# schmidtjonathan/pnmol-experiments

Measured on AMD Instinct MI355X. Metric: filter steps/sec, 1D heat N=512 nu=2 (white-noise EK1 predict+update), higher is better.
Workload: dtype f64; 1 GPU; 1-D heat equation, N=512 mesh, IWP(nu=2) EK1, Dirichlet, dt=2^-7, one problem per GPU (kappa sweep), D=1536, m=514; steps_in_one_call=4975, valid=True, problems_per_gpu=1

## Files before the change

pnmol-experiments_amd/csrc/pnmol_hip.hip:

```cpp
#include <hip/hip_runtime.h>

#include <algorithm>
#include <chrono>
#include <cmath>
#include <cstdio>
#include <cstdlib>
#include <cstring>
#include <string>
#include <utility>
#include <atomic>
#include <vector>

#include "pnmol_hip.h"
#include "pnmol_internal.hpp"

namespace {

constexpr int TLD = NB + 1;
typedef double d4 __attribute__((ext_vector_type(4)));

struct MeasModel {
    const int* ell_col;
    const double* ell_val;
    int w, d, m, dp, mp;
    double c0, c1;
};

constexpr int HW = 4;

struct HRow {
    int idx[HW + 1];
    double cf[HW + 1];
};

__device__ __forceinline__ void h_row_load(const MeasModel& mm, int i, HRow& r) {
    r.idx[0] = (i < mm.d) ? mm.dp + i : 0;
    r.cf[0] = (i < mm.d) ? mm.c1 : 0.0;
#pragma unroll
    for (int e = 0; e < HW; ++e) {
        const int cidx = (e < mm.w) ? mm.ell_col[e * mm.mp + i] : -1;
        const double val = (e < mm.w) ? mm.ell_val[e * mm.mp + i] : 0.0;
        r.idx[e + 1] = cidx >= 0 ? cidx : 0;
        r.cf[e + 1] = cidx >= 0 ? mm.c0 * val : 0.0;
    }
}

template <typename XT>
__device__ __forceinline__ double h_row_dot(const MeasModel& mm, int i, const XT* x) {
    double v = 0.0;
    if (i < mm.d) v = mm.c1 * x[mm.dp + i];
    for (int e = 0; e < mm.w; ++e) {
        const int cidx = mm.ell_col[e * mm.mp + i];
        if (cidx >= 0) v += mm.c0 * mm.ell_val[e * mm.mp + i] * x[cidx];
    }
    return v;
}

template <int W, typename XT>
__device__ __forceinline__ double h_row_dot_w(const HRow& r, const XT* __restrict__ x) {
    double xv[W + 1];
#pragma unroll
    for (int e = 0; e <= W; ++e) xv[e] = x[r.idx[e]];
    double v = r.cf[0] * xv[0];
#pragma unroll
    for (int e = 1; e <= W; ++e) v += r.cf[e] * xv[e];
    return v;
}

struct RoleArgs {
    IwpConsts c;
    int dp;
    const double* min;
    double* mpred;
    const double* shift;
    double* G;
    double* zbuf;
    MeasModel mm;
    int* flags;
    int nflags;
};

template <int N>
__device__ __forceinline__ void predict_vectors(double* mpl, int tid, const IwpConsts& c, int dp, const double* __restrict__ min,
                                                double* __restrict__ mpred, const double* __restrict__ shift,
                                                double* __restrict__ G, double* __restrict__ zbuf, const MeasModel& mm,
                                                int* __restrict__ flags, int nflags) {
    const long Dp = (long)N * dp;
    for (int e = tid; e < nflags; e += 256) flags[e] = 0;
    for (int j = tid; j < dp; j += 256) {
        double x[N];
#pragma unroll
        for (int a = 0; a < N; ++a) x[a] = c.ts[a] * min[a * dp + j];
#pragma unroll
        for (int a = 0; a < N; ++a) {
            double sacc = 0.0;
#pragma unroll
            for (int q = 0; q < N; ++q) sacc += c.A1[a * MAXN + q] * x[q];
            mpl[a * dp + j] = sacc;
            mpred[a * dp + j] = sacc;
        }
    }
    __syncthreads();
    for (int i = tid; i < mm.mp; i += 256) {
        const double v = (i < mm.m) ? h_row_dot(mm, i, mpl) + shift[i] : 0.0;
        G[((long)mm.mp + Dp) * mm.mp + i] = v;
        zbuf[i] = v;
    }
}

template <int N, typename PT>
__device__ __forceinline__ void predict_tile(const PT* __restrict__ Pin, PT* __restrict__ Pout, const double* __restrict__ Kg,
                                             const IwpConsts& c, int dp, int j, int k) {
    const long Dp = (long)N * dp;
    double X[N][N];
#pragma unroll
    for (int a = 0; a < N; ++a)
#pragma unroll
        for (int b = 0; b < N; ++b) X[a][b] = c.ts[a] * c.ts[b] * Pin[((long)a * dp + j) * Dp + (long)b * dp + k];
    const double kjk = Kg[(long)j * dp + k];
    double T[N][N];
#pragma unroll
    for (int a = 0; a < N; ++a)
#pragma unroll
        for (int e = 0; e < N; ++e) {
            double sacc = 0.0;
#pragma unroll
            for (int q = 0; q < N; ++q) sacc += c.A1[a * MAXN + q] * X[q][e];
            T[a][e] = sacc;
        }
#pragma unroll
    for (int a = 0; a < N; ++a)
#pragma unroll
        for (int b = 0; b < N; ++b) {
            double sacc = c.Q1[a * MAXN + b] * kjk;
#pragma unroll
            for (int e = 0; e < N; ++e) sacc += T[a][e] * c.A1[b * MAXN + e];
            Pout[((long)a * dp + j) * Dp + (long)b * dp + k] = (PT)sacc;
        }
}

template <int N>
__global__ __launch_bounds__(256) void k_predict(const void* __restrict__ Pin, void* __restrict__ Pout,
                                                 const double* __restrict__ Kg, IwpConsts c, int dp,
                                                 const double* __restrict__ min, double* __restrict__ mpred,
                                                 const double* __restrict__ shift, double* __restrict__ G,
                                                 double* __restrict__ zbuf, MeasModel mm, int* __restrict__ ctr,
                                                 int* __restrict__ flags, int nflags, int p32) {
    if (blockIdx.y == 0) {
        if (blockIdx.x != 0) return;
        extern __shared__ double mpl[];
        const int tid = threadIdx.y * 32 + threadIdx.x;
        predict_vectors<N>(mpl, tid, c, dp, min, mpred, shift, G, zbuf, mm, flags, nflags);
        if (tid == 0) *ctr += 1;
        return;
    }
    const int k = blockIdx.x * 32 + threadIdx.x;
    const int j = (blockIdx.y - 1) * 8 + threadIdx.y;
    if (p32) predict_tile<N>(static_cast<const float*>(Pin), static_cast<float*>(Pout), Kg, c, dp, j, k);
    else predict_tile<N>(static_cast<const double*>(Pin), static_cast<double*>(Pout), Kg, c, dp, j, k);
}

template <typename PT>
__device__ __forceinline__ double s_entry(const PT* __restrict__ Ppred, long Dp, const MeasModel& mm, int ip, int i,
                                          const double* __restrict__ rdiag, const double* __restrict__ Rdense) {
    if (ip >= mm.m || i >= mm.m) return (ip == i) ? 1.0 : 0.0;
    double v = 0.0;
    if (ip < mm.d) v = mm.c1 * h_row_dot(mm, i, Ppred + (long)(mm.dp + ip) * Dp);
    for (int e = 0; e < mm.w; ++e) {
        const int cidx = mm.ell_col[e * mm.mp + ip];
        if (cidx >= 0) v += mm.c0 * mm.ell_val[e * mm.mp + ip] * h_row_dot(mm, i, Ppred + (long)cidx * Dp);
    }
    if (ip == i) v += rdiag[i];
    if (Rdense) v += Rdense[(long)ip * mm.mp + i];
    return v;
}

template <int W, typename PT>
__device__ __forceinline__ double s_entry_w(const PT* __restrict__ Ppred, long Dp, const MeasModel& mm,
                                            const HRow& rrow , const HRow& rcol , int ip, int i,
                                            const double* __restrict__ rdiag, const double* __restrict__ Rdense) {
    if (ip >= mm.m || i >= mm.m) return (ip == i) ? 1.0 : 0.0;
    double t[W + 1];
#pragma unroll
    for (int e = 0; e <= W; ++e) t[e] = h_row_dot_w<W>(rcol, Ppred + (long)rrow.idx[e] * Dp);
    double v = rrow.cf[0] * t[0];
#pragma unroll
    for (int e = 1; e <= W; ++e) v += rrow.cf[e] * t[e];
    if (ip == i) v += rdiag[i];
    if (Rdense) v += Rdense[(long)ip * mm.mp + i];
    return v;
}

__device__ __forceinline__ double bcast_lane(double x, int src) {
    const int lo = __builtin_amdgcn_readlane(__double2loint(x), src);
    const int hi = __builtin_amdgcn_readlane(__double2hiint(x), src);
    return __hiloint2double(hi, lo);
}


struct Diag4Lds {
    double x0[4][64];
    double x1[8][64];
    double la[8][64];
    double n01[4][64];
    double piv[NB];
// ... 253 lines not shown
template <typename PT>
__device__ __forceinline__ void front_block_tiled(const PT* __restrict__ Ppred, double* __restrict__ G,
                                                  const double* __restrict__ rdiag, const double* __restrict__ Rdense,
                                                  const MeasModel& mm, long Dp, int fb) {
    const int tid = threadIdx.x, mp = mm.mp;
    const bool narrow = mm.w <= HW;
    const int nP = (int)(Dp / 8);
    if (fb < nP) {
        const long y0 = (long)fb * 8;
        for (int i = tid; i < mp; i += 256) {
            if (i >= mm.m) {
#pragma unroll
                for (int q = 0; q < 8; ++q) G[((long)mp + y0 + q) * mp + i] = 0.0;
                continue;
            }
            double v[8];
            if (narrow) {
                HRow rc;
                h_row_load(mm, i, rc);
#pragma unroll
                for (int q = 0; q < 8; ++q) v[q] = h_row_dot_w<HW>(rc, Ppred + (y0 + q) * Dp);
            } else {
#pragma unroll
                for (int q = 0; q < 8; ++q) v[q] = h_row_dot(mm, i, Ppred + (y0 + q) * Dp);
            }
#pragma unroll
            for (int q = 0; q < 8; ++q) G[((long)mp + y0 + q) * mp + i] = v[q];
        }
        return;
    }
    int t = fb - nP;
    int I = (int)((sqrt(8.0 * t + 1.0) - 1.0) * 0.5);
    while ((I + 1) * (I + 2) / 2 <= t) ++I;
    while (I * (I + 1) / 2 > t) --I;
    const int J = t - I * (I + 1) / 2;
    const int i = J * NB + (tid & 31);
    HRow rc;
    if (narrow && i < mm.m) h_row_load(mm, i, rc);
#pragma unroll
    for (int q = 0; q < 4; ++q) {
        const int ip = I * NB + (tid >> 5) + 8 * q;
        double v;
        if (narrow && ip < mm.m && i < mm.m) {
            HRow rr;
            h_row_load(mm, ip, rr);
            v = s_entry_w<HW>(Ppred, Dp, mm, rr, rc, ip, i, rdiag, Rdense);
        } else {
            v = s_entry(Ppred, Dp, mm, ip, i, rdiag, Rdense);
        }
        G[(long)ip * mp + i] = v;
    }
}

__global__ void k_set_identity(double* __restrict__ Gi, int mp) {
    const int q = blockIdx.x * blockDim.x + threadIdx.x;
    if (q < mp) Gi[(long)q * mp + q] = 1.0;
}

__global__ __launch_bounds__(256) void k_front(const void* __restrict__ Ppred, double* __restrict__ G,
                                               const double* __restrict__ rdiag, const double* __restrict__ Rdense,
                                               MeasModel mm, long Dp, int p32) {
    if (p32) front_block(static_cast<const float*>(Ppred), G, rdiag, Rdense, mm, Dp, blockIdx.x, blockIdx.y);
    else front_block(static_cast<const double*>(Ppred), G, rdiag, Rdense, mm, Dp, blockIdx.x, blockIdx.y);
}

__global__ __launch_bounds__(256) void k_front_s(double* __restrict__ G, const double* __restrict__ rdiag,
                                                 const double* __restrict__ Rdense, MeasModel mm) {
    const int i = blockIdx.x * 256 + threadIdx.x, ip = blockIdx.y, mp = mm.mp;
    if (i >= mp || i >= (ip / NB + 1) * NB) return;
    double v;
    if (ip >= mm.m || i >= mm.m) {
        v = (ip == i) ? 1.0 : 0.0;
    } else {
        const double* PHt = G + (long)mp * mp;
        v = 0.0;
        if (ip < mm.d) v = mm.c1 * PHt[(long)(mm.dp + ip) * mp + i];
        for (int e = 0; e < mm.w; ++e) {
            const int cidx = mm.ell_col[e * mp + ip];
            if (cidx >= 0) v += mm.c0 * mm.ell_val[e * mp + ip] * PHt[(long)cidx * mp + i];
        }
        if (ip == i) v += rdiag[i];
        if (Rdense) v += Rdense[(long)ip * mp + i];
    }
    G[(long)ip * mp + i] = v;
}

constexpr int SWEEP_SPIN_LIMIT = 1 << 18;
#ifdef PNMOL_SWEEP_STAMP
__device__ long long pnmol_sweep_stamp[512][8];
#define SWEEP_STAMP(slot) do { if (tid == 0 && L.stamp_id < 256) pnmol_sweep_stamp[L.stamp_id][slot] = wall_clock64(); } while (0)
#define SWEEP_STAMP_L(slot) do { if (l == 0 && L.stamp_id < 256) pnmol_sweep_stamp[L.stamp_id][slot] = wall_clock64(); } while (0)
#ifndef PNMOL_SWEEP_TRACE_WG
#define PNMOL_SWEEP_TRACE_WG 16
#endif
#define SWEEP_TRACE(j, slot) do { if (tid == 0 && L.stamp_id == PNMOL_SWEEP_TRACE_WG) pnmol_sweep_stamp[256 + (j)][slot] = wall_clock64(); } while (0)
#define SWEEP_TRACE_W2(j, slot) do { if (w == 2 && l == 0 && L.stamp_id == PNMOL_SWEEP_TRACE_WG) pnmol_sweep_stamp[320 + (j)][slot] = wall_clock64(); } while (0)
#define SWEEP_TRACE_VM(j, slot) do { asm volatile("s_waitcnt vmcnt(0)" ::: "memory"); SWEEP_TRACE(j, slot); } while (0)
#define CHAIN_TRACE(J, slot) do { if (tid == 0) pnmol_sweep_stamp[384 + (J)][slot] = wall_clock64(); } while (0)
#define CHAIN_TRACE_W(J, slot, wave) do { if (l == 0 && w == (wave)) pnmol_sweep_stamp[384 + (J)][slot] = wall_clock64(); } while (0)
#define CHAIN_TRACE_CLK(J, slot) do { if (tid == 0) pnmol_sweep_stamp[384 + (J)][slot] = clock64(); } while (0)
#define PNMOL_DD_DBG 1
#define DD_TRACE(j, slot) do { if (tid == 0 && pair == 60) pnmol_sweep_stamp[448 + (j)][slot] = wall_clock64(); } while (0)
#else
#define DD_TRACE(j, slot) do {} while (0)
#define CHAIN_TRACE_CLK(J, slot) do {} while (0)
#define SWEEP_TRACE_VM(j, slot) do {} while (0)
// ... 1729 lines not shown
    __syncthreads();
    if (w >= 2) return;
    {
        const double* rd = smem + w * C::RED;
#pragma unroll
        for (int a = 0; a < N; ++a)
#pragma unroll
            for (int b = 0; b < N; ++b)
#pragma unroll
                for (int r = 0; r < 4; ++r) acc[a][b][r] += rd[((a * N + b) * 4 + r) * 64 + l];
    }
    __syncthreads();
    if (w == 0)
        downdate_finish<N, 0>(acc, smem, Ppred, Pout, var, dp, Dp, J, K, l);
    else
        downdate_finish<N, 1>(acc, smem, Ppred, Pout, var, dp, Dp, J, K, l);
}

__global__ __launch_bounds__(256) void k_fill_q(void* __restrict__ Qf, const double* __restrict__ Kg, IwpConsts c, int n,
                                                int dp, int p32) {
    const long Dp = (long)n * dp;
    const long e = (long)blockIdx.x * 256 + threadIdx.x;
    if (e >= Dp * Dp) return;
    const long row = e / Dp, col = e % Dp;
    const int a = (int)(row / dp), j = (int)(row % dp), b = (int)(col / dp), k = (int)(col % dp);
    const double v = c.Q1[a * MAXN + b] * Kg[(long)j * dp + k];
    if (p32) static_cast<float*>(Qf)[e] = (float)v;
    else static_cast<double*>(Qf)[e] = v;
}

__global__ __launch_bounds__(256) void k_ttt(const double* __restrict__ T, double* __restrict__ C, int mp) {
    __shared__ double sa[16][17], sb[16][17];
    const int tx = threadIdx.x & 15, ty = threadIdx.x >> 4;
    const int i = blockIdx.y * 16 + ty, k = blockIdx.x * 16 + tx;
    double acc = 0.0;
    for (int q0 = 0; q0 < mp; q0 += 16) {
        sa[ty][tx] = T[(long)(blockIdx.y * 16 + ty) * mp + q0 + tx];
        sb[ty][tx] = T[(long)(blockIdx.x * 16 + ty) * mp + q0 + tx];
        __syncthreads();
#pragma unroll
        for (int q = 0; q < 16; ++q) acc += sa[ty][q] * sb[tx][q];
        __syncthreads();
    }
    C[(long)i * mp + k] = acc;
}

template <int N, bool ROLE>
__global__ __launch_bounds__(256) void k_readout(const double* __restrict__ mean, const double* __restrict__ var,
                                                 double* __restrict__ means_base, double* __restrict__ stds_base,
                                                 double s0, int d, const double* __restrict__ part,
                                                 double* __restrict__ rec_base, int mp, int* __restrict__ ctr,
                                                 RoleArgs ra, int* __restrict__ tickets, int rblocks,
                                                 const void* __restrict__ Ppred, const double* __restrict__ rdiag,
                                                 const double* __restrict__ Rdense, int p32) {
    if constexpr (ROLE) {
        if ((int)blockIdx.x > rblocks) {
            const int fb = blockIdx.x - rblocks - 1;
            if (p32) front_block_tiled(static_cast<const float*>(Ppred), ra.G, rdiag, Rdense, ra.mm, (long)N * ra.dp, fb);
            else front_block_tiled(static_cast<const double*>(Ppred), ra.G, rdiag, Rdense, ra.mm, (long)N * ra.dp, fb);
            return;
        }
    }
    const int slot = __builtin_amdgcn_readfirstlane(*ctr) - 1;
    if constexpr (ROLE) {
        if ((int)blockIdx.x == rblocks) {
            extern __shared__ double mpl[];
            predict_vectors<N>(mpl, threadIdx.x, ra.c, ra.dp, ra.min, ra.mpred, ra.shift, ra.G, ra.zbuf, ra.mm, ra.flags,
                               ra.nflags);
            if (threadIdx.x == 0) {
                int spins = 0;
                while (__hip_atomic_load(tickets, __ATOMIC_RELAXED, __HIP_MEMORY_SCOPE_AGENT) < rblocks &&
                       ++spins < (1 << 22)) __builtin_amdgcn_s_sleep(1);
                *ctr = slot + 2;
                __hip_atomic_store(tickets, 0, __ATOMIC_RELAXED, __HIP_MEMORY_SCOPE_AGENT);
            }
            return;
        }
        __syncthreads();
        if (threadIdx.x == 0) atomicAdd(tickets, 1);
    }
    const int j = blockIdx.x * blockDim.x + threadIdx.x;
    double* means = means_base ? means_base + (size_t)slot * d : nullptr;
    double* stds = stds_base ? stds_base + (size_t)slot * d : nullptr;
    double* rec = rec_base + 4 * (size_t)slot;
    if (j < d) {
        if (means) means[j] = s0 * mean[j];
        if (stds) stds[j] = s0 * sqrt(fmax(var[j], 0.0));
    }
    if (blockIdx.x == 0) {
        __shared__ double sred[3][4];
        double a[3] = {0.0, 0.0, 0.0};
        for (int i = threadIdx.x; i < mp; i += 256)
#pragma unroll
            for (int q = 0; q < 3; ++q) a[q] += part[q * mp + i];
#pragma unroll
        for (int q = 0; q < 3; ++q)
#pragma unroll
            for (int o = 32; o > 0; o >>= 1) a[q] += __shfl_xor(a[q], o);
        if ((threadIdx.x & 63) == 0)
            for (int q = 0; q < 3; ++q) sred[q][threadIdx.x >> 6] = a[q];
        __syncthreads();
        if (threadIdx.x < 3) rec[threadIdx.x] = sred[threadIdx.x][0] + sred[threadIdx.x][1] + sred[threadIdx.x][2] + sred[threadIdx.x][3];
    }
}

__global__ __launch_bounds__(256) void k_poison(double* __restrict__ F, long nF, double* __restrict__ Linv, long nL,
                                                double* __restrict__ hs, long nH) {
    const double bad = __longlong_as_double(0x7ff8dead0000beefLL);
    const long stride = (long)gridDim.x * 256;
    for (long e = (long)blockIdx.x * 256 + threadIdx.x; e < nF; e += stride) F[e] = bad;
    for (long e = (long)blockIdx.x * 256 + threadIdx.x; e < nL; e += stride) {
        const int r = (int)((e / NB) % NB), c = (int)(e % NB);
        if (!(r < 16 && c >= 16)) Linv[e] = bad;
    }
    for (long e = (long)blockIdx.x * 256 + threadIdx.x; e < nH; e += stride) hs[e] = bad;
}

__global__ void k_operator_diagonal(double* __restrict__ ell_val, const double* __restrict__ base_val,
                                    const int* __restrict__ slot, const double* __restrict__ op ,
                                    double* __restrict__ shift, int d, int mp) {
    const int i = blockIdx.x * blockDim.x + threadIdx.x;
// ... 199 lines not shown
    static const int mode = [] {
        const char* e = std::getenv("PNMOL_HIP_SWEEP_XL");
        return e ? (std::atoi(e) != 0 ? 1 : 0) : -1;
    }();
    return mode;
}
constexpr int MAX_DEVICES = 64;
std::atomic<int> live_rl_filters[MAX_DEVICES];
template <int N, bool FUSED>
void launch_sweep(unsigned grid, hipStream_t st, const double* G, double* F, double* Linv, int ld, int CB, int RT, int* flags,
                  int* info, const int* ctr, const DowndateArgs& dd, int* claim, double* hs, int lenient, int home,
                  bool wskip = false) {
    const bool xl = home >= 0;
    const unsigned rgrid = grid + (unsigned)w_split_count(RT, CB);
    unsigned xgrid = 8u * (unsigned)(CB - 1 + s_split_count(CB, true)) + 1u;
    for (unsigned left = rgrid - (unsigned)CB; left > 0; ++xgrid)
        if (xgrid % 8u != 0u) --left;
    xgrid += (unsigned)(xl ? home : 0);
    if (sweep_rl_enabled() && CB <= 9) {
        if (xl) k_sweep_rl<N, FUSED, 9, true><<<xgrid, 256, 0, st>>>(G, F, Linv, ld, CB, RT, flags, info, ctr, dd, hs, lenient, home);
        else k_sweep_rl<N, FUSED, 9, false><<<rgrid + 1, 256, 0, st>>>(G, F, Linv, ld, CB, RT, flags, info, ctr, dd, hs, lenient, home);
    } else if (sweep_rl_enabled() && CB <= 17) {
        if (xl) k_sweep_rl<N, FUSED, 17, true><<<xgrid, 256, 0, st>>>(G, F, Linv, ld, CB, RT, flags, info, ctr, dd, hs, lenient, home);
        else k_sweep_rl<N, FUSED, 17, false><<<rgrid + 1, 256, 0, st>>>(G, F, Linv, ld, CB, RT, flags, info, ctr, dd, hs, lenient, home);
    }
    else
        k_sweep<N, FUSED><<<grid, 256, 0, st>>>(G, F, Linv, ld, CB, RT, flags, info, ctr, dd, claim, hs, lenient, wskip ? 1 : 0);
}

inline bool short_last_panel() {
    static const int on = [] {
        const char* e = std::getenv("PNMOL_HIP_SHORT_LAST");
        return e ? std::atoi(e) : 1;
    }();
    return on != 0;
}
template <int N>
int launch_step(pnmol_filter* f, const double* Pin, const double* min, double frame_dt, double dt, double* Pout,
                double* mout, double* varout, bool record, StepKind kind) {
    pnmol_ctx* ctx = f->ctx;
    hipStream_t st = ctx->stream;
    IwpConsts c = f->iwp;
    for (int a = 0; a < f->n; ++a) {
        const double so = frame_dt == 0.0 ? 1.0 : nordsieck_scale(f->nu, a, frame_dt);
        c.ts[a] = so / nordsieck_scale(f->nu, a, dt);
    }
    MeasModel mm{f->ell_col, f->ell_val, f->ellw, f->d, f->m, f->dp, f->mp,
                 nordsieck_scale(f->nu, 0, dt), nordsieck_scale(f->nu, 1, dt)};
    const int dp = f->dp, mp = f->mp;
    const long Dp = f->Dp;

    if (kind != STEP_STEADY)
        k_predict<N><<<dim3(dp / 32, dp / 8 + 1), dim3(32, 8), sizeof(double) * Dp, st>>>(
        Pin, f->Ppred, f->Kg, c, dp, min, f->mpred, f->shift, f->G, f->zbuf, mm, f->ctr, f->flags, f->nflags, f->p32);
    if (kind != STEP_STEADY) {
        if (f->ellw > HW) {
            k_front<<<dim3((mp + 255) / 256, (unsigned)Dp), 256, 0, st>>>(f->Ppred, f->G, f->rdiag, f->Rdense, mm, Dp, f->p32);
            k_front_s<<<dim3((mp + 255) / 256, (unsigned)mp), 256, 0, st>>>(f->G, f->rdiag, f->Rdense, mm);
        } else {
            k_front<<<dim3((mp + 255) / 256, (unsigned)(Dp + mp)), 256, 0, st>>>(f->Ppred, f->G, f->rdiag, f->Rdense, mm, Dp, f->p32);
        }
    }
    const long rowI0 = (long)mp + Dp + NB;
    const double* W = f->F + (long)mp * mp;
    const bool have_sq = (f->Sqinv != nullptr && f->sq_dt == dt);
    VecArgs va{f->mpred, f->F + ((long)mp + Dp) * mp, f->F + rowI0 * mp, f->zbuf, have_sq ? f->Sqinv : nullptr,
               mout, f->part};
    const int nreal = f->m - NB * (f->CB - 1);
    DowndateArgs dd{f->Ppred, Pout, varout, dp, 0, va, kind == STEP_FULL ? nullptr : f->Ppred, f->Kg, f->last_ctr, {}, {}, f->p32,
                    (nreal < 8 && short_last_panel()) ? nreal : 0};
    std::memcpy(dd.A1, f->iwp.A1, sizeof(dd.A1));
    std::memcpy(dd.Q1, f->iwp.Q1, sizeof(dd.Q1));
    if (f->sweep_mode == 2) {
        const int t32 = dp / NB, pairs = t32 * (t32 + 1) / 2;
        dd.vrows = 0;
        if constexpr (N <= 3)
            launch_sweep<N, true>(f->RT + pairs, st, f->G, f->F, f->Linv, mp, f->CB, f->RT, f->flags, f->info, f->ctr, dd,
                                  f->flags + f->RT + f->CB + 1, f->hs_scratch, f->p32 ? 2 : 0, f->xcd_home);
    } else {
        if (f->w_gemm) {
            launch_sweep<N, false>(2 * f->CB + 1, st, f->G, f->F, f->Linv, mp, f->CB, f->RT, f->flags, f->info, f->ctr, dd,
                                   f->flags + f->RT + f->CB + 1, f->hs_scratch, f->p32 ? 2 : 0, f->xcd_home, true);
            const int nI = (int)(Dp / BDT), nt = nI * (mp / BDT);
            k_w_gemm<<<8 * ((nt + 7) / 8), 256, 0, st>>>(f->G + (long)mp * mp, f->F + rowI0 * mp, f->F + (long)mp * mp, mp, nI, nt);
        } else
        launch_sweep<N, false>(f->RT, st, f->G, f->F, f->Linv, mp, f->CB, f->RT, f->flags, f->info, f->ctr, dd,
                               f->flags + f->RT + f->CB + 1, f->hs_scratch, f->p32 ? 2 : 0, f->xcd_home);
        const int tiles = dp / 16;
        const int vrows = (int)(((Dp + mp + 3) / 4 + tiles - 1) / tiles);
        if (f->dd_big) {
            const int T = (int)(Dp / BDT), nt = T * (T + 1) / 2;
            if (f->p32)
                k_downdate_big<float><<<8 * ((nt + 7) / 8), 256, 0, st>>>(reinterpret_cast<const float*>(f->Ppred), W,
                                                                          reinterpret_cast<float*>(Pout), varout, Dp, mp, nt);
            else
                k_downdate_big<double><<<8 * ((nt + 7) / 8), 256, 0, st>>>(static_cast<const double*>(f->Ppred), W, Pout, varout,
                                                                           Dp, mp, nt);
            k_vecops<<<dim3(tiles, vrows), 256, 0, st>>>(va, W, mp, Dp, tiles);
        } else {
            k_downdate<N><<<dim3(tiles, tiles + vrows), 256, 0, st>>>(f->Ppred, W, Pout, varout, dp, mp, 0, mp / 8, va);
        }
    }
    IwpConsts cn = f->iwp;
    for (int a = 0; a < MAXN; ++a) cn.ts[a] = 1.0;
    RoleArgs ra{cn, dp, mout, f->mpred, f->shift, f->G, f->zbuf, mm, f->flags, f->nflags};
    const unsigned rblocks = (f->d + 255) / 256;
    if (kind == STEP_FULL)
        k_readout<N, false><<<rblocks, 256, 0, st>>>(mout, varout, record ? f->rec_means : nullptr,
                                                    record ? f->rec_stds : nullptr, nordsieck_scale(f->nu, 0, dt), f->d,
                                                    f->part, f->rec, mp, f->ctr, ra, f->tickets, (int)rblocks, f->Ppred, f->rdiag,
                                                    f->Rdense, f->p32);
    else
        k_readout<N, true><<<rblocks + 1 + (unsigned)front_tiled_blocks(Dp, mp), 256, sizeof(double) * Dp, st>>>(
            mout, varout, record ? f->rec_means : nullptr, record ? f->rec_stds : nullptr, nordsieck_scale(f->nu, 0, dt),
            f->d, f->part, f->rec, mp, f->ctr, ra, f->tickets, (int)rblocks, f->Ppred, f->rdiag, f->Rdense, f->p32);
    hipError_t e = hipGetLastError();
    if (e != hipSuccess) {
        ctx->err = std::string("kernel launch: ") + hipGetErrorString(e);
        return -2;
    }
    return 0;
}

int dispatch_step(pnmol_filter* f, const double* Pin, const double* min, double frame_dt, double dt, double* Pout,
                  double* mout, double* varout, bool record, StepKind kind = STEP_FULL) {
    switch (f->n) {
        case 2: return launch_step<2>(f, Pin, min, frame_dt, dt, Pout, mout, varout, record, kind);
        case 3: return launch_step<3>(f, Pin, min, frame_dt, dt, Pout, mout, varout, record, kind);
        case 4: return launch_step<4>(f, Pin, min, frame_dt, dt, Pout, mout, varout, record, kind);
    }
    return -1;
}

int loop_step(pnmol_filter* f, const double* Pin, const double* min, double frame_dt, double dt, double* Pout, double* mout,
              double* varout, StepKind kind, bool keep = true) {
    if (has_term(f)) {
        if (int rc = pnmol_reaction_enqueue(f, min, frame_dt, dt, true)) return rc;
    }
    if (int rc = dispatch_step(f, Pin, min, frame_dt, dt, Pout, mout, varout, true, kind)) return rc;
    return keep ? pnmol_record_enqueue(f, Pout, mout, varout) : 0;
}

void drop_graphs(pnmol_filter* f) {
    for (auto& g : f->graphs)
        if (g.exec) (void)hipGraphExecDestroy(g.exec);
    f->graphs.clear();
}

int get_graph(pnmol_filter* f, double* P0, double* M0, double* P1, double* M1, double* var, double dt, int nsteps,
              hipGraphExec_t* out) {
    pnmol_ctx* ctx = f->ctx;
    const bool have_sq = (f->Sqinv != nullptr && f->sq_dt == dt);
    for (auto& g : f->graphs)
        if (g.P0 == P0 && g.P1 == P1 && g.var == var && g.dt == dt && g.nsteps == nsteps && g.have_sq == have_sq &&
            g.fused == fused_loop(f)) {
            *out = g.exec;
            return 0;
        }
    if (f->graphs.size() >= 8) drop_graphs(f);
    hipGraph_t graph = nullptr;
    HIPCHK(ctx, hipStreamBeginCapture(ctx->stream, hipStreamCaptureModeThreadLocal));
    int rc = 0;
    for (int it = 0; it < nsteps && rc == 0; ++it)
        rc = (it & 1) ? loop_step(f, P1, M1, dt, dt, P0, M0, var, fused_loop(f) ? STEP_STEADY : STEP_FULL)
                      : loop_step(f, P0, M0, dt, dt, P1, M1, var, fused_loop(f) ? STEP_STEADY : STEP_FULL);
    hipError_t e = hipStreamEndCapture(ctx->stream, &graph);
    if (rc != 0 || e != hipSuccess) {
        if (graph) (void)hipGraphDestroy(graph);
// ... 387 lines not shown
    FCHK(hipMalloc(&f->ell_val, sizeof(double) * eval.size()));
    FCHK(hipMalloc(&f->Kg, sizeof(double) * Kg.size()));
    FCHK(hipMalloc(&f->rdiag, sizeof(double) * mp));
    FCHK(hipMalloc(&f->shift, sizeof(double) * mp));
    FCHK(hipMalloc(&f->G, sizeof(double) * tall));
    FCHK(hipMalloc(&f->F, sizeof(double) * tall));
    FCHK(hipMalloc(&f->Linv, sizeof(double) * (size_t)f->CB * NB * NB));
    FCHK(hipMemset(f->Linv, 0, sizeof(double) * (size_t)f->CB * NB * NB));
    FCHK(hipMalloc(&f->Ppred, f->psz * (size_t)Dp * Dp));
    FCHK(hipMalloc(&f->tmpP, f->psz * (size_t)Dp * Dp));
    FCHK(hipMalloc(&f->mpred, sizeof(double) * Dp));
    FCHK(hipMalloc(&f->tmpMean, sizeof(double) * Dp));
    FCHK(hipMalloc(&f->var, sizeof(double) * Dp));
    FCHK(hipMalloc(&f->zbuf, sizeof(double) * mp));
    FCHK(hipMalloc(&f->part, sizeof(double) * 3 * mp));
    FCHK(hipMalloc(&f->ctr, sizeof(int)));
    {
        const int h1 = 1;
        FCHK(hipMalloc(&f->one, sizeof(int)));
        FCHK(hipMalloc(&f->info_err, sizeof(int)));
        FCHK(hipMemcpy(f->one, &h1, sizeof(int), hipMemcpyHostToDevice));
    }
    if (const char* gc = std::getenv("PNMOL_HIP_GRAPH_CHUNK")) f->graph_chunk = std::atoi(gc) / 2 * 2;
    f->sweep_mode = sweep_mode;
    if (f->sweep_mode == 2 && n > 3) f->sweep_mode = 1;
    {
        const char* e = std::getenv("PNMOL_HIP_DD_BIG");
        const bool fits = f->Dp % BDT == 0 && f->mp % BDK == 0 && (!f->p32 || f->sweep_mode == 2);
        const bool want = e ? std::atoi(e) != 0 : (f->Dp >= 8192 && f->CB > 17);
        if (fits && want) {
            f->dd_big = 1;
            f->sweep_mode = 1;
            const char* g = std::getenv("PNMOL_HIP_W_GEMM");
            f->w_gemm = (g ? std::atoi(g) != 0 : 1) && f->mp % BDT == 0 && f->CB > 17;
        }
    }
    {
        static std::atomic<int> next_home[MAX_DEVICES];
        const bool rl = sweep_rl_enabled() && f->CB <= 17;
        if (rl) {
            const int dv = ctx->device % MAX_DEVICES;
            const int others = live_rl_filters[dv].fetch_add(1);
            f->counted = true;
            const bool xl = sweep_xl_mode() < 0 ? others == 0 : sweep_xl_mode() == 1;
            f->xcd_home = xl ? next_home[dv].fetch_add(1) % 8 : -1;
        }
    }
    f->nflags = std::max({f->RT + f->CB + 1 + f->CB * f->CB, rl_flags(f->RT, f->CB).total,
                          rl_flags((int)(f->Dp / NB) + 1, (int)(f->Dp / NB) + 1).total});
    FCHK(hipMalloc(&f->flags, sizeof(int) * f->nflags));
    FCHK(hipMemset(f->flags, 0, sizeof(int) * f->nflags));
    FCHK(hipMalloc(&f->hs_scratch, sizeof(double) * (size_t)std::max(f->CB * f->CB, 2 * f->CB + 2) * NB * NB));
    if (const char* e = std::getenv("PNMOL_HIP_FUSE_PREDICT")) f->fuse_predict = std::atoi(e);
    FCHK(hipMalloc(&f->last_ctr, sizeof(int)));
    FCHK(hipMemset(f->last_ctr, 0, sizeof(int)));
    FCHK(hipMalloc(&f->tickets, sizeof(int)));
    FCHK(hipMemset(f->tickets, 0, sizeof(int)));
    if (f->p32 && f->sweep_mode != 2 && !f->dd_big) {
        ctx->err = "pnmol_filter_create: dtype = fp32 covariance needs the fused sweep (num_derivatives <= 2, PNMOL_HIP_SWEEP unset)";
        return fail(-1);
    }
    FCHK(hipMemcpy(f->ell_col, ecol.data(), sizeof(int) * ecol.size(), hipMemcpyHostToDevice));
    FCHK(hipMemcpy(f->ell_val, eval.data(), sizeof(double) * eval.size(), hipMemcpyHostToDevice));
    {
        std::vector<int> slot((size_t)mp, 0);
        f->base_has_diag = 1;
        for (int i = 0; i < d; ++i) {
            int e = 0;
            while (e < w && ecol[(size_t)e * mp + i] != i) ++e;
            if (e == w) f->base_has_diag = 0, e = 0;
            slot[i] = e;
        }
        f->base_w = w;
        FCHK(hipMalloc(&f->ell_col_base, sizeof(int) * ecol.size()));
        FCHK(hipMalloc(&f->ell_val_base, sizeof(double) * eval.size()));
        FCHK(hipMalloc(&f->ell_diag_slot, sizeof(int) * mp));
        FCHK(hipMemcpy(f->ell_col_base, ecol.data(), sizeof(int) * ecol.size(), hipMemcpyHostToDevice));
        FCHK(hipMemcpy(f->ell_val_base, eval.data(), sizeof(double) * eval.size(), hipMemcpyHostToDevice));
        FCHK(hipMemcpy(f->ell_diag_slot, slot.data(), sizeof(int) * mp, hipMemcpyHostToDevice));
        FCHK(hipHostMalloc(&f->h_op, sizeof(double) * (size_t)(d + mp), hipHostMallocMapped));
        FCHK(hipHostGetDevicePointer(reinterpret_cast<void**>(&f->h_op_dev), f->h_op, 0));
        FCHK(hipEventCreate(&f->ev_op));
    }
    FCHK(hipMemcpy(f->Kg, Kg.data(), sizeof(double) * Kg.size(), hipMemcpyHostToDevice));
    FCHK(hipMemcpy(f->rdiag, rdiag.data(), sizeof(double) * mp, hipMemcpyHostToDevice));
    if (!diag) {
        FCHK(hipMalloc(&f->Rdense, sizeof(double) * Rd.size()));
        FCHK(hipMemcpy(f->Rdense, Rd.data(), sizeof(double) * Rd.size(), hipMemcpyHostToDevice));
    }
    FCHK(hipMemset(f->shift, 0, sizeof(double) * mp));
    FCHK(hipMemset(f->G, 0, sizeof(double) * tall));
    k_set_identity<<<(mp + 255) / 256, 256>>>(f->G + ((size_t)mp + Dp + NB) * mp, mp);
    FCHK(hipDeviceSynchronize());
    FCHK(hipMemset(f->F, 0, sizeof(double) * tall));
    FCHK(hipMemset(f->var, 0, sizeof(double) * Dp));
    FCHK(hipMemset(f->tmpP, 0, f->psz * (size_t)Dp * Dp));
    FCHK(hipMemset(f->tmpMean, 0, sizeof(double) * Dp));
    FCHK(hipEventCreate(&f->ev0));
    FCHK(hipEventCreate(&f->ev1));
#undef FCHK
    if (ensure_rec(f, 128) != 0) return fail(-2);
    *out = f;
    return 0;
}

int pnmol_filter_destroy(pnmol_filter* f) {
// ... 483 lines not shown
```

pnmol-experiments_amd/csrc/pnmol_internal.hpp:

```cpp
#pragma once
#include <hip/hip_runtime.h>

#include <algorithm>
#include <atomic>
#include <cmath>
#include <string>
#include <vector>

#include "pnmol_hip.h"
#include "pnmol_observe_plan.hpp"

constexpr int NB = 32;
constexpr int MAXN = 4;

namespace {
struct IwpConsts {
    double A1[MAXN * MAXN];
    double Q1[MAXN * MAXN];
    double ts[MAXN];
};
}

#define HIPCHK(ctx, call)                                                                        \
    do {                                                                                         \
// ... 6 lines not shown

inline int round_up(int x, int q) { return (x + q - 1) / q * q; }

inline double nordsieck_scale(int nu, int a, double dt) {
    double fact = 1.0;
    for (int q = 2; q <= nu - a; ++q) fact *= q;
    return std::pow(std::fabs(dt), nu - a + 0.5) / fact;
}

struct pnmol_ctx {
    int device = 0;
    hipStream_t stream = nullptr;
    std::string err;
    std::atomic<int> children{0};
};

struct SweepWs {
    double *G = nullptr, *F = nullptr, *Linv = nullptr, *feed = nullptr;
    int *flags = nullptr, *info = nullptr;
    int nflags = 0;
    int rt = 0, cb = 0, ld = 0;
    bool left_looking = false;
};
hipError_t sweep_ws_alloc(SweepWs* w, pnmol_ctx* ctx, int rt, int cb);
void sweep_ws_free(SweepWs* w);
int sweep_ws_enqueue(pnmol_filter* f, const SweepWs& w, hipStream_t st, int lenient, const char* who);
int sweep_info_result(pnmol_ctx* ctx, int inf, long limit, const char* who, const char* what,
                      const char* wait = "a dependency wait timed out");

struct ObserveWs {
    int qp = 0;
    SweepWs sweep;
    double* dev = nullptr;
    std::vector<double> host;
};

enum class TermKind { none, scalar, system, convection };
struct TermImage {
    int* col = nullptr;
    double* val = nullptr;
    double* g = nullptr;
    int* slot = nullptr;
    int w = 0, slot_rows = 0;
    TermKind kind = TermKind::none;
    int ncomp = 0;
};

struct pnmol_filter {
    pnmol_ctx* ctx = nullptr;
    int d = 0, n = 0, nu = 0, nB = 0, m = 0, dp = 0, mp = 0, CB = 0, RBS = 0, RBW = 0, RT = 0, ellw = 0;
    int* tickets = nullptr;
    int* last_ctr = nullptr;
    int fuse_predict = 1;
    int* flags = nullptr;
    int nflags = 0;
    double* hs_scratch = nullptr;
    int w_gemm = 0;
    int dd_big = 0;
    int sweep_mode = 2;
    int ds = 0;
    bool counted = false;
    bool registered = false;
    std::atomic<int> states{0};
    int xcd_home = -1;
    int p32 = 0;
    size_t psz = 8;
    long Dp = 0;
    IwpConsts iwp{};
    int* ell_col = nullptr;
    double* ell_val = nullptr;
    int* ell_col_base = nullptr;
    double* ell_val_base = nullptr;
    int* ell_diag_slot = nullptr;
    int base_w = 0, base_has_diag = 0;
    int ell_is_base = 1;
    double* h_op = nullptr;
    double* h_op_dev = nullptr;
    hipEvent_t ev_op = nullptr;
    double *Kg = nullptr, *rdiag = nullptr, *Rdense = nullptr, *shift = nullptr;
    double *G = nullptr, *F = nullptr, *Linv = nullptr, *Ppred = nullptr, *mpred = nullptr, *zbuf = nullptr;
    double *var = nullptr, *Sqinv = nullptr, *rec = nullptr, *part = nullptr;
    int* info = nullptr;
    std::vector<double> sqdiag;
    double* Qfull = nullptr;
    int* one = nullptr;
    int* info_err = nullptr;
    double sq_dt = -1.0;
    std::vector<double> hB;
    int ell_cap = 0;
    double *tmpP = nullptr, *tmpMean = nullptr;
    double *rec_means = nullptr, *rec_stds = nullptr;
    double* h_pin = nullptr;
    double* h_pin_dev = nullptr;
    int rec_cap = 0;
    hipEvent_t ev0 = nullptr, ev1 = nullptr;
    float last_ms = 0.f;
    int* ctr = nullptr;
    int pending_k = 0;
    double pending_dt = 0.0;
    pnmol_state* pending_state = nullptr;
    struct GraphEntry {
        double *P0, *P1, *var;
        double dt;
        int nsteps;
        bool have_sq;
        bool fused;
// ... 165 lines not shown
```

Before: 8124 steps/s.

## Add slab-based front kernel staging shared H*P rows in LDS

Adds a new front path, on by default, for forming the innovation covariance S = H P H^T + R and the H P rows. Each S block first collects the unique P rows its H rows reference, computes H·row once per unique row into an LDS slab, then assembles S entries from that slab instead of recomputing h_row_dot for every (ip, i) pair. Row blocks are split into separate 64-row tiles. The predict_vectors mean observation also gains a narrow path that preloads ELL rows into registers in batches of four and uses a fixed-order FMA dot product. The new path needs more LDS per block and adds atomics and syncthreads for deduplication, which could lower occupancy.

```diff
diff --git a/pnmol-experiments_amd/csrc/pnmol_hip.hip b/pnmol-experiments_amd/csrc/pnmol_hip.hip
--- a/pnmol-experiments_amd/csrc/pnmol_hip.hip
+++ b/pnmol-experiments_amd/csrc/pnmol_hip.hip
@@ -64,6 +64,18 @@
     double v = r.cf[0] * xv[0];
 #pragma unroll
     for (int e = 1; e <= W; ++e) v += r.cf[e] * xv[e];
+    return v;
+}
+
+template <int W, typename XT>
+__device__ __forceinline__ double h_row_dot_seq(const HRow& r, const XT* x) {
+#pragma clang fp contract(off)
+    double xv[W + 1];
+#pragma unroll
+    for (int e = 0; e <= W; ++e) xv[e] = x[r.idx[e]];
+    double v = r.cf[0] * xv[0];
+#pragma unroll
+    for (int e = 1; e <= W; ++e) v = __builtin_fma(r.cf[e], xv[e], v);
     return v;
 }
 
@@ -80,12 +92,45 @@
     int nflags;
 };
 
+constexpr int PVC = 4;
 template <int N>
 __device__ __forceinline__ void predict_vectors(double* mpl, int tid, const IwpConsts& c, int dp, const double* __restrict__ min,
                                                 double* __restrict__ mpred, const double* __restrict__ shift,
                                                 double* __restrict__ G, double* __restrict__ zbuf, const MeasModel& mm,
-                                                int* __restrict__ flags, int nflags) {
+                                                int* __restrict__ flags, int nflags, bool pre) {
     const long Dp = (long)N * dp;
+    const bool narrow = pre && mm.w <= HW;
+    HRow hr[PVC];
+    double sh[PVC];
+    auto load_rows = [&](int base) {
+        int col[PVC][HW];
+        double val[PVC][HW];
+#pragma unroll
+        for (int e = 0; e < HW; ++e)
+#pragma unroll
+            for (int q = 0; q < PVC; ++q) {
+                const int i = base + tid + 256 * q, ic = i < mm.m ? i : 0;
+                col[q][e] = (e < mm.w) ? mm.ell_col[e * mm.mp + ic] : -1;
+                val[q][e] = (e < mm.w) ? mm.ell_val[e * mm.mp + ic] : 0.0;
+            }
+#pragma unroll
+        for (int q = 0; q < PVC; ++q) {
+            const int i = base + tid + 256 * q;
+            sh[q] = shift[i < mm.m ? i : 0];
+        }
+#pragma unroll
+        for (int q = 0; q < PVC; ++q) {
+            const int i = base + tid + 256 * q;
+            hr[q].idx[0] = (i < mm.d) ? mm.dp + i : 0;
+            hr[q].cf[0] = (i < mm.d) ? mm.c1 : 0.0;
+#pragma unroll
+            for (int e = 0; e < HW; ++e) {
+                hr[q].idx[e + 1] = col[q][e] >= 0 ? col[q][e] : 0;
+                hr[q].cf[e + 1] = col[q][e] >= 0 ? mm.c0 * val[q][e] : 0.0;
+            }
+        }
+    };
+    if (narrow) load_rows(0);
     for (int e = tid; e < nflags; e += 256) flags[e] = 0;
     for (int j = tid; j < dp; j += 256) {
         double x[N];
@@ -101,6 +146,21 @@
         }
     }
     __syncthreads();
+    if (narrow) {
+        for (int base = 0; base < mm.mp; base += 256 * PVC) {
+            if (base) load_rows(base);
+#pragma unroll
+            for (int q = 0; q < PVC; ++q) {
+                const int i = base + tid + 256 * q;
+                if (i < mm.mp) {
+                    const double v = (i < mm.m) ? h_row_dot_seq<HW>(hr[q], mpl) + sh[q] : 0.0;
+                    G[((long)mm.mp + Dp) * mm.mp + i] = v;
+                    zbuf[i] = v;
+                }
+            }
+        }
+        return;
+    }
     for (int i = tid; i < mm.mp; i += 256) {
         const double v = (i < mm.m) ? h_row_dot(mm, i, mpl) + shift[i] : 0.0;
         G[((long)mm.mp + Dp) * mm.mp + i] = v;
@@ -145,12 +205,12 @@
                                                  const double* __restrict__ min, double* __restrict__ mpred,
                                                  const double* __restrict__ shift, double* __restrict__ G,
                                                  double* __restrict__ zbuf, MeasModel mm, int* __restrict__ ctr,
-                                                 int* __restrict__ flags, int nflags, int p32) {
+                                                 int* __restrict__ flags, int nflags, int p32, int pre) {
     if (blockIdx.y == 0) {
         if (blockIdx.x != 0) return;
         extern __shared__ double mpl[];
         const int tid = threadIdx.y * 32 + threadIdx.x;
-        predict_vectors<N>(mpl, tid, c, dp, min, mpred, shift, G, zbuf, mm, flags, nflags);
+        predict_vectors<N>(mpl, tid, c, dp, min, mpred, shift, G, zbuf, mm, flags, nflags, pre != 0);
         if (tid == 0) *ctr += 1;
         return;
     }
@@ -510,6 +570,162 @@
     }
 }
 
+constexpr int FS_ROWS = 16, FS_PAIRS = FS_ROWS * (HW + 1), FS_CAP = 40, FR_ROWS = 64;
+constexpr int FS_TAIL = FS_PAIRS * 8 + FS_CAP * 4 + FS_PAIRS * 4 + 16;
+__host__ __device__ inline long front_slab_region(long Dp) { return Dp / 2 > FS_CAP * NB ? Dp / 2 : FS_CAP * NB; }
+inline size_t front_slab_lds(long Dp) {
+    const size_t need = sizeof(double) * (size_t)front_slab_region(Dp) + FS_TAIL;
+    return std::max(sizeof(double) * (size_t)Dp, need);
+}
+__host__ __device__ inline int front_slab_s_blocks(int mp) { return (mp / NB) * (mp / NB + 1); }
+__host__ __device__ inline int front_slab_blocks(long Dp, int mp) {
+    return front_slab_s_blocks(mp) + (int)((Dp + FR_ROWS - 1) / FR_ROWS) * (mp / NB);
+}
+
+template <typename PT>
+__device__ __forceinline__ void front_rows_slab(const PT* __restrict__ Ppred, double* __restrict__ G, const MeasModel& mm, long Dp,
+                                                int rb) {
+    const int tid = threadIdx.x, mp = mm.mp, CB = mp / NB;
+    const int c = tid & 31, g = tid >> 5;
+    const int i = (rb % CB) * NB + c;
+    const long y0 = (long)(rb / CB) * FR_ROWS;
+    const bool narrow = mm.w <= HW, real = i < mm.m;
+    HRow rc;
+    if (narrow) h_row_load(mm, real ? i : 0, rc);
+    double v[FR_ROWS / 8];
+#pragma unroll
+    for (int k = 0; k < FR_ROWS / 8; ++k) {
+        const long y = y0 + g + 8 * k;
+        const PT* row = Ppred + (y < Dp ? y : y0) * Dp;
+        if (narrow) v[k] = h_row_dot_w<HW>(rc, row);
+        else v[k] = real ? h_row_dot(mm, i, row) : 0.0;
+    }
+#pragma unroll
+    for (int k = 0; k < FR_ROWS / 8; ++k) {
+        const long y = y0 + g + 8 * k;
+        if (y < Dp) G[((long)mp + y) * mp + i] = real ? v[k] : 0.0;
+    }
+}
+
+template <typename PT>
+__device__ __forceinline__ void front_s_slab(const PT* __restrict__ Ppred, double* __restrict__ G,
+                                             const double* __restrict__ rdiag, const double* __restrict__ Rdense,
+                                             const MeasModel& mm, long Dp, int sb, double* lds) {
+    const int tid = threadIdx.x, mp = mm.mp;
+    const int t = sb >> 1;
+    int I = (int)((sqrt(8.0 * t + 1.0) - 1.0) * 0.5);
+    while ((I + 1) * (I + 2) / 2 <= t) ++I;
+    while (I * (I + 1) / 2 > t) --I;
+    const int J = t - I * (I + 1) / 2;
+    const int c = tid & 31, g = tid >> 5;
+    const int i = J * NB + c, ip0 = I * NB + (sb & 1) * FS_ROWS;
+    if (mm.w > HW) {
+#pragma unroll
+        for (int q = 0; q < FS_ROWS / 8; ++q) {
+            const int ip = ip0 + g + 8 * q;
+            G[(long)ip * mp + i] = s_entry(Ppred, Dp, mm, ip, i, rdiag, Rdense);
+        }
+        return;
+    }
+    double* slab = lds;
+    int* tbl = reinterpret_cast<int*>(lds);
+    double* scf = lds + front_slab_region(Dp);
+    int* srow = reinterpret_cast<int*>(scf + FS_PAIRS);
+    int* sidx = srow + FS_CAP;
+    int* scnt = sidx + FS_PAIRS;
+
+    const int ic = i < mm.m ? i : 0;
+    const int pip = ip0 + (tid < FS_PAIRS ? tid : 0) / (HW + 1), pe = (tid < FS_PAIRS ? tid : 0) % (HW + 1) - 1;
+    const bool pslot = pe >= 0 && pe < mm.w;
+    const int praw = mm.ell_col[(pslot ? pe : 0) * mp + (pip < mm.m ? pip : 0)];
+    const double pval = mm.ell_val[(pslot ? pe : 0) * mp + (pip < mm.m ? pip : 0)];
+    const double rdi = rdiag[ic];
+    double rn[FS_ROWS / 8];
+#pragma unroll
+    for (int q = 0; q < FS_ROWS / 8; ++q) {
+        const int ip = ip0 + g + 8 * q;
+        rn[q] = Rdense ? Rdense[(long)(ip < mm.m ? ip : 0) * mp + ic] : 0.0;
+    }
+    HRow rc;
+    h_row_load(mm, ic, rc);
+    int py = -1;
+    double pcf = 0.0;
+    if (tid < FS_PAIRS && pip < mm.m) {
+        if (pe < 0) {
+            py = (pip < mm.d) ? mm.dp + pip : 0;
+            pcf = (pip < mm.d) ? mm.c1 : 0.0;
+        } else {
+            const int cidx = pslot ? praw : -1;
+            py = cidx >= 0 ? cidx : 0;
+            pcf = cidx >= 0 ? mm.c0 * pval : 0.0;
+        }
+    }
+
+    for (long k = tid; k < Dp; k += 256) tbl[k] = 0x7fffffff;
+    __syncthreads();
+    if (py >= 0) atomicMin(&tbl[py], tid);
+    if (tid < FS_PAIRS) scf[tid] = pcf;
+    __syncthreads();
+    const bool lead = py >= 0 && tbl[py] == tid;
+    const unsigned long long leaders = __ballot(lead);
+    const int lane = tid & 63, wv = tid >> 6;
+    if (lane == 0 && wv < 2) scnt[wv] = __popcll(leaders);
+    __syncthreads();
+    const int total = scnt[0] + scnt[1];
+    const int nslab = total < FS_CAP ? total : FS_CAP;
+    if (lead) {
+        const int rank = (wv == 1 ? scnt[0] : 0) + __popcll(leaders & ((1ull << lane) - 1ull));
+        tbl[py] = rank < FS_CAP ? rank : -1;
+        if (rank < FS_CAP) srow[rank] = py;
+    }
+    __syncthreads();
+    if (tid < FS_PAIRS) sidx[tid] = py >= 0 ? tbl[py] : -1;
+
+    double v[FS_CAP / 8];
+#pragma unroll
+    for (int k = 0; k < FS_CAP / 8; ++k) {
+        const int r = g + 8 * k;
+        const long y = r < nslab ? srow[r] : 0;
+        v[k] = h_row_dot_w<HW>(rc, Ppred + y * Dp);
+    }
+    __syncthreads();
+#pragma unroll
+    for (int k = 0; k < FS_CAP / 8; ++k) slab[(g + 8 * k) * NB + c] = v[k];
+    __syncthreads();
+
+#pragma unroll
+    for (int q = 0; q < FS_ROWS / 8; ++q) {
+        const int ipl = g + 8 * q, ip = ip0 + ipl;
+        double s;
+        if (ip >= mm.m || i >= mm.m) {
+            s = (ip == i) ? 1.0 : 0.0;
+        } else {
+            int si[HW + 1];
+            bool in = true;
+#pragma unroll
+            for (int e = 0; e <= HW; ++e) {
+                si[e] = sidx[ipl * (HW + 1) + e];
+                in = in && si[e] >= 0;
+            }
+            if (in) {
+                double tt[HW + 1];
+#pragma unroll
+                for (int e = 0; e <= HW; ++e) tt[e] = slab[si[e] * NB + c];
+                s = scf[ipl * (HW + 1)] * tt[0];
+#pragma unroll
+                for (int e = 1; e <= HW; ++e) s += scf[ipl * (HW + 1) + e] * tt[e];
+                if (ip == i) s += rdi;
+                if (Rdense) s += rn[q];
+            } else {
+                HRow rr;
+                h_row_load(mm, ip, rr);
+                s = s_entry_w<HW>(Ppred, Dp, mm, rr, rc, ip, i, rdiag, Rdense);
+            }
+        }
+        G[(long)ip * mp + i] = s;
+    }
+}
+
 __global__ void k_set_identity(double* __restrict__ Gi, int mp) {
     const int q = blockIdx.x * blockDim.x + threadIdx.x;
     if (q < mp) Gi[(long)q * mp + q] = 1.0;
@@ -2345,10 +2561,23 @@
                                                  double* __restrict__ rec_base, int mp, int* __restrict__ ctr,
                                                  RoleArgs ra, int* __restrict__ tickets, int rblocks,
                                                  const void* __restrict__ Ppred, const double* __restrict__ rdiag,
-                                                 const double* __restrict__ Rdense, int p32) {
+                                                 const double* __restrict__ Rdense, int p32, int slab) {
     if constexpr (ROLE) {
         if ((int)blockIdx.x > rblocks) {
             const int fb = blockIdx.x - rblocks - 1;
+            if (slab) {
+                extern __shared__ double flds[];
+                const long Dp = (long)N * ra.dp;
+                const int ns = front_slab_s_blocks(ra.mm.mp);
+                if (fb < ns) {
+                    if (p32) front_s_slab(static_cast<const float*>(Ppred), ra.G, rdiag, Rdense, ra.mm, Dp, fb, flds);
+                    else front_s_slab(static_cast<const double*>(Ppred), ra.G, rdiag, Rdense, ra.mm, Dp, fb, flds);
+                } else {
+                    if (p32) front_rows_slab(static_cast<const float*>(Ppred), ra.G, ra.mm, Dp, fb - ns);
+                    else front_rows_slab(static_cast<const double*>(Ppred), ra.G, ra.mm, Dp, fb - ns);
+                }
+                return;
+            }
             if (p32) front_block_tiled(static_cast<const float*>(Ppred), ra.G, rdiag, Rdense, ra.mm, (long)N * ra.dp, fb);
             else front_block_tiled(static_cast<const double*>(Ppred), ra.G, rdiag, Rdense, ra.mm, (long)N * ra.dp, fb);
             return;
@@ -2359,7 +2588,7 @@
         if ((int)blockIdx.x == rblocks) {
             extern __shared__ double mpl[];
             predict_vectors<N>(mpl, threadIdx.x, ra.c, ra.dp, ra.min, ra.mpred, ra.shift, ra.G, ra.zbuf, ra.mm, ra.flags,
-                               ra.nflags);
+                               ra.nflags, slab != 0);
             if (threadIdx.x == 0) {
                 int spins = 0;
                 while (__hip_atomic_load(tickets, __ATOMIC_RELAXED, __HIP_MEMORY_SCOPE_AGENT) < rblocks &&
@@ -2665,7 +2894,8 @@
 
     if (kind != STEP_STEADY)
         k_predict<N><<<dim3(dp / 32, dp / 8 + 1), dim3(32, 8), sizeof(double) * Dp, st>>>(
-        Pin, f->Ppred, f->Kg, c, dp, min, f->mpred, f->shift, f->G, f->zbuf, mm, f->ctr, f->flags, f->nflags, f->p32);
+        Pin, f->Ppred, f->Kg, c, dp, min, f->mpred, f->shift, f->G, f->zbuf, mm, f->ctr, f->flags, f->nflags, f->p32,
+        f->front_slab);
     if (kind != STEP_STEADY) {
         if (f->ellw > HW) {
             k_front<<<dim3((mp + 255) / 256, (unsigned)Dp), 256, 0, st>>>(f->Ppred, f->G, f->rdiag, f->Rdense, mm, Dp, f->p32);
@@ -2722,11 +2952,15 @@
         k_readout<N, false><<<rblocks, 256, 0, st>>>(mout, varout, record ? f->rec_means : nullptr,
                                                     record ? f->rec_stds : nullptr, nordsieck_scale(f->nu, 0, dt), f->d,
                                                     f->part, f->rec, mp, f->ctr, ra, f->tickets, (int)rblocks, f->Ppred, f->rdiag,
-                                                    f->Rdense, f->p32);
-    else
-        k_readout<N, true><<<rblocks + 1 + (unsigned)front_tiled_blocks(Dp, mp), 256, sizeof(double) * Dp, st>>>(
+                                                    f->Rdense, f->p32, 0);
+    else {
+        const unsigned fblocks = (unsigned)(f->front_slab ? front_slab_blocks(Dp, mp) : front_tiled_blocks(Dp, mp));
+        const size_t lds = f->front_slab ? front_slab_lds(Dp) : sizeof(double) * Dp;
+        k_readout<N, true><<<rblocks + 1 + fblocks, 256, lds, st>>>(
             mout, varout, record ? f->rec_means : nullptr, record ? f->rec_stds : nullptr, nordsieck_scale(f->nu, 0, dt),
-            f->d, f->part, f->rec, mp, f->ctr, ra, f->tickets, (int)rblocks, f->Ppred, f->rdiag, f->Rdense, f->p32);
+            f->d, f->part, f->rec, mp, f->ctr, ra, f->tickets, (int)rblocks, f->Ppred, f->rdiag, f->Rdense, f->p32,
+            f->front_slab);
+    }
     hipError_t e = hipGetLastError();
     if (e != hipSuccess) {
         ctx->err = std::string("kernel launch: ") + hipGetErrorString(e);
@@ -3220,6 +3454,7 @@
     FCHK(hipMemset(f->flags, 0, sizeof(int) * f->nflags));
     FCHK(hipMalloc(&f->hs_scratch, sizeof(double) * (size_t)std::max(f->CB * f->CB, 2 * f->CB + 2) * NB * NB));
     if (const char* e = std::getenv("PNMOL_HIP_FUSE_PREDICT")) f->fuse_predict = std::atoi(e);
+    if (const char* e = std::getenv("PNMOL_HIP_FRONT_SLAB")) f->front_slab = std::atoi(e) != 0;
     FCHK(hipMalloc(&f->last_ctr, sizeof(int)));
     FCHK(hipMemset(f->last_ctr, 0, sizeof(int)));
     FCHK(hipMalloc(&f->tickets, sizeof(int)));
diff --git a/pnmol-experiments_amd/csrc/pnmol_internal.hpp b/pnmol-experiments_amd/csrc/pnmol_internal.hpp
--- a/pnmol-experiments_amd/csrc/pnmol_internal.hpp
+++ b/pnmol-experiments_amd/csrc/pnmol_internal.hpp
@@ -82,6 +82,7 @@
     int* tickets = nullptr;
     int* last_ctr = nullptr;
     int fuse_predict = 1;
+    int front_slab = 1;
     int* flags = nullptr;
     int nflags = 0;
     double* hs_scratch = nullptr;
```

After: 8256 steps/s (median of 6 runs). No clear change (+1.6%).
